# kerry-he/fsae-mpc

Hardware: AMD Instinct MI355X
Metric: QP solves/sec (batched LTV-MPC, N=40 nx=5 nu=2 fp64) (higher is better)
Workload: dtype f64

## Files before the change

### fsae-mpc_amd/csrc/qp_solve_kernel.h

```cpp
#pragma once
#include "qp_solver.h"
#include "qp_lane.h"

#ifndef QP_SOLVE_PAIR
#define QP_SOLVE_PAIR 0
#endif
#ifndef QP_DIAG_FLAT
#define QP_DIAG_FLAT 1
#endif
#ifndef QP_SYRK_INTERLEAVE
#define QP_SYRK_INTERLEAVE 0
#endif
#ifndef QP_STARTUP_ATW
#define QP_STARTUP_ATW 0
#endif

namespace {

template <int T> struct Tri {
  static constexpr int NT = T * (T + 1) / 2;
  __host__ __device__ static constexpr int idx(int I, int J) { return I * T - (I * (I - 1)) / 2 + (J - I); }
};

struct Ctx {
  int n, m, T, Kq, J, JB, JT, np, lane, c, q, nc, nb, ntr;
  const int* perm; const int* tcs; const int* aoff; const int* tend;
  const double* Aw; const double* Hw; const double* Ab; const double* Hb;
  double* rows;
  double* ring;
  double* cof;
  int rowlen;
  double* vec;
};
enum VecArr { V_X = 0, V_G, V_HX, V_R1, V_R2, V_P1, V_P2, V_P3, V_DX, V_E, V_NARR };

DEVINL double* rowp(const Ctx& k, int arr) { return k.rows + (size_t)arr * k.rowlen; }
DEVINL double* vecp(const Ctx& k, int arr) { return k.vec + arr * k.np; }

DEVINL bool row_valid(const Ctx& k, int js) {
  if (js < k.J) { const int s = 16 * js + k.c; return s < k.Kq && 4 * s + k.q < k.m; }
  return (js - k.J) * 64 + k.lane < k.n;
}

template <int T> DEVINL void hx_tiles(const Ctx& k, const double* X, double* HX) {
  double hx[T], hn[T][4], hc[T][4];
#pragma unroll
  for (int t = 0; t < T; ++t) hx[t] = 0.0;
#pragma unroll
  for (int Jt = 0; Jt < T; ++Jt)
#pragma unroll
    for (int p = 0; p < 4; ++p) hn[Jt][p] = k.Hw[((size_t)Jt * 4 + p) * 64 + k.lane];
#pragma unroll 1
  for (int I = 0; I < T; ++I) {
#pragma unroll
    for (int Jt = 0; Jt < T; ++Jt)
#pragma unroll
      for (int p = 0; p < 4; ++p) hc[Jt][p] = hn[Jt][p];
    if (I + 1 < T) {
#pragma unroll
      for (int Jt = 0; Jt < T; ++Jt)
#pragma unroll
        for (int p = 0; p < 4; ++p) hn[Jt][p] = k.Hw[((size_t)((I + 1) * T + Jt) * 4 + p) * 64 + k.lane];
    }
    double xk[4];
#pragma unroll
    for (int p = 0; p < 4; ++p) xk[p] = X[16 * I + k.q + 4 * p];
#pragma unroll
    for (int Jt = 0; Jt < T; ++Jt)
#pragma unroll
      for (int p = 0; p < 4; ++p) hx[Jt] = fma(hc[Jt][p], xk[p], hx[Jt]);
  }
#pragma unroll
  for (int t = 0; t < T; ++t) {
    double v = q_sum(hx[t]);
    if (k.q == 0) HX[16 * t + k.c] = v;
  }
}
template <int T> DEVINL void acc_init(const Ctx& k, v4d* acc) {
#pragma unroll
  for (int I = 0; I < T; ++I)
#pragma unroll
    for (int Jt = I; Jt < T; ++Jt) {
      const double* hp = k.Hw + ((size_t)(I * T + Jt) * 4) * 64 + k.lane;
      v4d h;
#pragma unroll
      for (int p = 0; p < 4; ++p) h[p] = hp[p * 64];
      acc[Tri<T>::idx(I, Jt)] = h;
    }
}

template <int T> DEVINL void hx_from_acc(const Ctx& k, const v4d* acc, const double* XV, double* HX) {
  double xr[T][4], xc[T], sc[T], sr[T][4];
#pragma unroll
  for (int I = 0; I < T; ++I) {
    xc[I] = XV[16 * I + k.c]; sc[I] = 0.0;
#pragma unroll
    for (int p = 0; p < 4; ++p) { xr[I][p] = XV[16 * I + k.q + 4 * p]; sr[I][p] = 0.0; }
  }
#pragma unroll
  for (int I = 0; I < T; ++I)
#pragma unroll
    for (int J = I; J < T; ++J) {
      const v4d& h = acc[Tri<T>::idx(I, J)];
#pragma unroll
      for (int p = 0; p < 4; ++p) {
        sc[J] = fma(h[p], xr[I][p], sc[J]);
        if (J > I) sr[I][p] = fma(h[p], xc[J], sr[I][p]);
      }
    }
  WAVE_SYNC();
#pragma unroll
  for (int J = 0; J < T; ++J) { const double v = q_sum(sc[J]); if (k.q == 0) HX[16 * J + k.c] = v; }
  WAVE_SYNC();
#pragma unroll
  for (int I = 0; I < T - 1; ++I) {
    grp16_sum(sr[I]);
#pragma unroll
    for (int p = 0; p < 4; ++p) if (k.c == 0) HX[16 * I + k.q + 4 * p] += sr[I][p];
  }
}

template <int C> struct IC { static constexpr int value = C; };

template <int T> struct StreamCfg {
  static constexpr int D = 2 * T;
  static constexpr int R = D + T;
};
template <int T> struct Stream {
  static constexpr int D = StreamCfg<T>::D, R = StreamCfg<T>::R;
  static_assert(R == QP_SOLVE_RING(T), "qp_solve_lds (qp_solver.h) sizes the ring");
  const char* gnext; int slot_i, slot_e;
  int tend[T + 1];
  DEVINL void issue(const Ctx& k) {
    __builtin_amdgcn_global_load_lds((const __attribute__((address_space(1))) void*)(gnext + k.lane * 16),
                                     (__attribute__((address_space(3))) void*)(k.ring + slot_i * 128), 16, 0, 0);
    gnext += 1024;
    slot_i = slot_i + 1 == R ? 0 : slot_i + 1;
  }
  DEVINL void open(const Ctx& k) {
    gnext = reinterpret_cast<const char*>(k.Aw); slot_i = 0; slot_e = 0;
#pragma unroll
    for (int C = 0; C <= T; ++C) tend[C] = uni(k.tend[C]);
  }
  DEVINL void start(const Ctx& k) {
    gnext = reinterpret_cast<const char*>(k.Aw); slot_i = 0; slot_e = 0;
    if (k.ntr > 0) {
#pragma unroll
      for (int j = 0; j < D; ++j) issue(k);
    }
#pragma unroll
    for (int C = 0; C <= T; ++C) tend[C] = uni(tend[C]);
  }
  template <int C> DEVINL void next_pair(const Ctx& k, v2d* b) {
#pragma unroll
    for (int t = 0; t < C; ++t) issue(k);
    asm volatile("s_waitcnt vmcnt(%0)" :: "n"(D) : "memory");
#pragma unroll
    for (int t = 0; t < C; ++t) {
      int sl = slot_e + t; if (sl >= R) sl -= R;
      b[t] = *reinterpret_cast<const v2d*>(k.ring + sl * 128 + k.lane * 2);
    }
    slot_e += C; if (slot_e >= R) slot_e -= R;
  }
  DEVINL void finish() { asm volatile("s_waitcnt vmcnt(0)" ::: "memory"); }
  DEVINL void close() { asm volatile("s_waitcnt vmcnt(0)" ::: "memory"); }
};

// ... 239 lines not shown
      double pv = q_sum(pc[t]);
      if (k.q == 0) Pcor[16 * t + k.c] = pv;
    }
#pragma unroll
    for (int f = 0; f < NB; ++f) { const double pv = q_sum(pcb[f]); if (k.lane == 0) Pcor[k.nc + f] = pv; }
  }
  if (FUSE >= 2) {
#pragma unroll
    for (int t = 0; t < T; ++t) {
      double pv = q_sum(pd[t]);
      if (k.q == 0) Pcor2[16 * t + k.c] = pv;
    }
#pragma unroll
    for (int f = 0; f < NB; ++f) { const double pv = q_sum(pdb[f]); if (k.lane == 0) Pcor2[k.nc + f] = pv; }
  }
}

template <int T, int NB> DEVINL void pass_Atw(const Ctx& k, const double* W, double* Pout) {
  constexpr int NBB = NB > 0 ? NB : 1;
  const int JS = k.J * 64;
  double p[T], pbv[NBB];
#pragma unroll
  for (int t = 0; t < T; ++t) p[t] = 0.0;
#pragma unroll
  for (int f = 0; f < NBB; ++f) pbv[f] = 0.0;
  for (int s = 0; s < 4 * k.ntr; ++s) {
    const int ri = (s >> 4) * 64 + k.q * 16 + (s & 15);
    const double w = W[ri];
    const int tr = s >> 2, tc = k.tcs[tr];
    const double* src = k.Aw + ((size_t)k.aoff[tr] + ((s >> 1) & 1) * tc) * 128 + k.lane * 2 + (s & 1);
#pragma unroll
    for (int t = 0; t < T; ++t)
      if (t < tc) p[t] = fma(w, src[t * 128], p[t]);
#pragma unroll
    for (int f = 0; f < NB; ++f) pbv[f] = fma(w, k.Ab[(size_t)f * JS + ri], pbv[f]);
  }
#pragma unroll
  for (int t = 0; t < T; ++t) {
    double v = q_sum(p[t]);
    if (k.q == 0) Pout[16 * t + k.c] = v;
  }
#pragma unroll
  for (int f = 0; f < NB; ++f) { const double pv = q_sum(pbv[f]); if (k.lane == 0) Pout[k.nc + f] = pv; }
}

template <int T> DEVINL void mfma4_sub(const v4d& X, const v4d& Y, v4d& Dst) {
#pragma unroll
  for (int p = 0; p < 4; ++p) Dst = __builtin_amdgcn_mfma_f64_16x16x4f64(-X[p], Y[p], Dst, 0, 0, 0);
}
DEVINL v4d mfma4_new(const v4d& X, const v4d& Y) {
  v4d Z = {0.0, 0.0, 0.0, 0.0};
#pragma unroll
  for (int p = 0; p < 4; ++p) Z = __builtin_amdgcn_mfma_f64_16x16x4f64(X[p], Y[p], Z, 0, 0, 0);
  return Z;
}

DEVINL void tile_store(const Ctx& k, double* slot, const v4d& Xt) {
#pragma unroll
  for (int p = 0; p < 4; ++p) slot[(k.q + 4 * p) * 17 + k.c] = Xt[p];
}
DEVINL v4d tile_load(const Ctx& k, const double* slot) {
  v4d Z;
#pragma unroll
  for (int p = 0; p < 4; ++p) Z[p] = slot[(k.q + 4 * p) * 17 + k.c];
  return Z;
}
DEVINL v4d tile_load_t(const Ctx& k, const double* slot) {
  v4d Z;
#pragma unroll
  for (int p = 0; p < 4; ++p) Z[p] = slot[k.c * 17 + k.q + 4 * p];
  return Z;
}

DEVINL double on_lanes(unsigned long long mask, double v, double otherwise) {
  return __builtin_amdgcn_inverse_ballot_w64(mask) ? v : otherwise;
}
template <int FORM> DEVINL int diag_factor(const Ctx& k, v4d& Ud, v4d& Yk, v4d& rk, double floor_abs) {
  constexpr bool FLAT = FORM >= 1;
  int bad = 0;
#pragma unroll
  for (int p = 0; p < 4; ++p) {
    const double d00 = rl(Ud[p], 4 * p + 0), d01 = rl(Ud[p], 4 * p + 1), d02 = rl(Ud[p], 4 * p + 2), d03 = rl(Ud[p], 4 * p + 3);
    const double d11 = rl(Ud[p], 16 + 4 * p + 1), d12 = rl(Ud[p], 16 + 4 * p + 2), d13 = rl(Ud[p], 16 + 4 * p + 3);
    const double d22 = rl(Ud[p], 32 + 4 * p + 2), d23 = rl(Ud[p], 32 + 4 * p + 3);
    const double d33 = rl(Ud[p], 48 + 4 * p + 3);
    auto piv = [&](double t) {
      if constexpr (FORM >= 2) {
        const bool low = !(t > floor_abs);
        bad |= (low & !(fabs(t) < INFINITY)) ? 1 : 0;
        t = low ? floor_abs : t;
      } else {
        if (!(t > floor_abs)) { if (!(fabs(t) < INFINITY)) bad = 1; t = floor_abs; }
      }
      return rsqrt(t);
    };
    const double i0 = piv(d00);
    const double r01 = d01 * i0, r02 = d02 * i0, r03 = d03 * i0;
    const double i1 = piv(fma(-r01, r01, d11));
    const double r12 = fma(-r01, r02, d12) * i1, r13 = fma(-r01, r03, d13) * i1;
    const double i2 = piv(fma(-r12, r12, fma(-r02, r02, d22)));
    const double r23 = fma(-r12, r13, fma(-r02, r03, d23)) * i2;
    const double i3 = piv(fma(-r23, r23, fma(-r13, r13, fma(-r03, r03, d33))));
    const double w10 = -r01 * i0 * i1;
    const double w20 = -fma(r12, w10, r02 * i0) * i2, w21 = -r12 * i1 * i2;
    const double w30 = -fma(r23, w20, fma(r13, w10, r03 * i0)) * i3, w31 = -fma(r23, w21, r13 * i1) * i3, w32 = -r23 * i2 * i3;
    const v4d z = {0.0, 0.0, 0.0, 0.0};
    if constexpr (FLAT) {
      const unsigned long long L0 = 1ull << (4 * p), L1 = 1ull << (16 + 4 * p), L2 = 1ull << (32 + 4 * p), L3 = 1ull << (48 + 4 * p);
      double wa = on_lanes(L0, i0, 0.0);
      wa = on_lanes(L0 << 1, w10, wa); wa = on_lanes(L0 << 2, w20, wa); wa = on_lanes(L0 << 3, w30, wa);
      wa = on_lanes(L1 << 1, i1, wa); wa = on_lanes(L1 << 2, w21, wa); wa = on_lanes(L1 << 3, w31, wa);
      wa = on_lanes(L2 << 2, i2, wa); wa = on_lanes(L2 << 3, w32, wa);
      wa = on_lanes(L3 << 3, i3, wa);
      const v4d nu = __builtin_amdgcn_mfma_f64_16x16x4f64(wa, Ud[p], z, 0, 0, 0);
      Ud[p] = nu[p];
      double a = 0.0;
      if (p < 3) {
        a = on_lanes(0x0001000100010001ull * (0xFFFFull & (0xFFFFull << (4 * p + 4))), -Ud[p], 0.0);
        Ud = __builtin_amdgcn_mfma_f64_16x16x4f64(a, Ud[p], Ud, 0, 0, 0);
      }
      const v4d ny = __builtin_amdgcn_mfma_f64_16x16x4f64(wa, Yk[p], z, 0, 0, 0);
      const v4d nr = __builtin_amdgcn_mfma_f64_16x16x4f64(wa, rk[p], z, 0, 0, 0);
      Yk[p] = ny[p]; rk[p] = nr[p];
      if (p < 3) {
        Yk = __builtin_amdgcn_mfma_f64_16x16x4f64(a, Yk[p], Yk, 0, 0, 0);
        rk = __builtin_amdgcn_mfma_f64_16x16x4f64(a, rk[p], rk, 0, 0, 0);
      }
      if constexpr (FORM >= 2) asm("" : "+v"(bad));
    } else {
      const int a_ = k.c - 4 * p;
      double wa = 0.0;
      if (k.q == 0) wa = a_ == 0 ? i0 : (a_ == 1 ? w10 : (a_ == 2 ? w20 : (a_ == 3 ? w30 : 0.0)));
      if (k.q == 1) wa = a_ == 1 ? i1 : (a_ == 2 ? w21 : (a_ == 3 ? w31 : 0.0));
      if (k.q == 2) wa = a_ == 2 ? i2 : (a_ == 3 ? w32 : 0.0);
      if (k.q == 3) wa = a_ == 3 ? i3 : 0.0;
      const v4d nu = __builtin_amdgcn_mfma_f64_16x16x4f64(wa, Ud[p], z, 0, 0, 0);
      const v4d ny = __builtin_amdgcn_mfma_f64_16x16x4f64(wa, Yk[p], z, 0, 0, 0);
      const v4d nr = __builtin_amdgcn_mfma_f64_16x16x4f64(wa, rk[p], z, 0, 0, 0);
      Ud[p] = nu[p]; Yk[p] = ny[p]; rk[p] = nr[p];
      if (p < 3) {
        const double a = (k.c > 4 * p + 3) ? -Ud[p] : 0.0;
        Yk = __builtin_amdgcn_mfma_f64_16x16x4f64(a, Yk[p], Yk, 0, 0, 0);
        rk = __builtin_amdgcn_mfma_f64_16x16x4f64(a, rk[p], rk, 0, 0, 0);
        Ud = __builtin_amdgcn_mfma_f64_16x16x4f64(a, Ud[p], Ud, 0, 0, 0);
      }
    }
  }
#pragma unroll
  for (int p = 0; p < 4; ++p) if (k.c < k.q + 4 * p) Ud[p] = 0.0;
  return bad;
}

template <int T, int NB> struct DiagForm { static constexpr int form = (T == 5 && NB > 0) ? QP_DIAG_FLAT : 0; };

template <int T, int NB, int K> struct FactorStep {
  static DEVINL int run(const Ctx& k, v4d* acc, double* YL, double floor_abs) {
    v4d Yk, none = {0.0, 0.0, 0.0, 0.0};
#pragma unroll
    for (int p = 0; p < 4; ++p) Yk[p] = (k.q + 4 * p == k.c) ? 1.0 : 0.0;
    int bad = diag_factor<DiagForm<T, NB>::form>(k, acc[Tri<T>::idx(K, K)], Yk, none, floor_abs);
    tile_store(k, YL + K * 272, Yk);
    WAVE_SYNC();
    const v4d Wk = tile_load_t(k, YL + K * 272);
    const v4d& UKK = acc[Tri<T>::idx(K, K)];
#pragma unroll
    for (int Jt = K + 1; Jt < T; ++Jt) {
      v4d Rr = acc[Tri<T>::idx(K, Jt)];
      v4d Ukj = mfma4_new(Wk, Rr);
      mfma4_sub<T>(UKK, Ukj, Rr);
#pragma unroll
      for (int p = 0; p < 4; ++p) Ukj = __builtin_amdgcn_mfma_f64_16x16x4f64(Wk[p], Rr[p], Ukj, 0, 0, 0);
      acc[Tri<T>::idx(K, Jt)] = Ukj;
    }
#pragma unroll
    for (int I = K + 1; I < T; ++I) {
      const v4d& UKI = acc[Tri<T>::idx(K, I)];
#pragma unroll
      for (int Jt = I; Jt < T; ++Jt) mfma4_sub<T>(UKI, acc[Tri<T>::idx(K, Jt)], acc[Tri<T>::idx(I, Jt)]);
    }
    return bad | FactorStep<T, NB, K + 1>::run(k, acc, YL, floor_abs);
  }
};
template <int T, int NB> struct FactorStep<T, NB, T> {
  static DEVINL int run(const Ctx&, v4d*, double*, double) { return 0; }
};
template <int T, int NB> DEVINL int reg_factor(const Ctx& k, v4d* acc, double* YL, double floor_abs) {
  return FactorStep<T, NB, 0>::run(k, acc, YL, floor_abs);
}

template <int T, bool REFINE, int NV> DEVINL void vec_forward(const Ctx& k, const v4d* acc, const double* YL, const double* const (&B)[NV], double (&y)[NV][T][4]) {
#pragma unroll
  for (int K = 0; K < T; ++K) {
    double s[NV], t[NV];
#pragma unroll
    for (int v = 0; v < NV; ++v) {
      s[v] = 0.0;
#pragma unroll
      for (int I = 0; I < K; ++I)
#pragma unroll
        for (int p = 0; p < 4; ++p) s[v] = fma(acc[Tri<T>::idx(I, K)][p], y[v][I][p], s[v]);
    }
    if (K > 0) q_sum(s);
#pragma unroll
    for (int v = 0; v < NV; ++v) t[v] = B[v][16 * K + k.c] - (K > 0 ? s[v] : 0.0);
    const v4d Yt = tile_load(k, YL + K * 272);
    double yk[NV * 4];
#pragma unroll
    for (int v = 0; v < NV; ++v)
#pragma unroll
      for (int p = 0; p < 4; ++p) yk[4 * v + p] = Yt[p] * t[v];
    grp16_sum(yk);
    if (REFINE) {
      const v4d& U = acc[Tri<T>::idx(K, K)];
      double r[NV], dy[NV * 4];
#pragma unroll
      for (int v = 0; v < NV; ++v) {
        r[v] = 0.0;
#pragma unroll
        for (int p = 0; p < 4; ++p) r[v] = fma(U[p], yk[4 * v + p], r[v]);
      }
      q_sum(r);
#pragma unroll
      for (int v = 0; v < NV; ++v) {
        r[v] = t[v] - r[v];
#pragma unroll
        for (int p = 0; p < 4; ++p) dy[4 * v + p] = Yt[p] * r[v];
      }
      grp16_sum(dy);
#pragma unroll
      for (int i = 0; i < NV * 4; ++i) yk[i] += dy[i];
    }
#pragma unroll
    for (int v = 0; v < NV; ++v)
#pragma unroll
      for (int p = 0; p < 4; ++p) y[v][K][p] = yk[4 * v + p];
  }
}
template <int T, bool REFINE> DEVINL void vec_forward(const Ctx& k, const v4d* acc, const double* YL, const double* B, double (&y)[T][4]) {
  const double* const b1[1] = {B};
  vec_forward<T, REFINE, 1>(k, acc, YL, b1, reinterpret_cast<double (&)[1][T][4]>(y));
}
template <int T, bool REFINE, int NV> DEVINL void vec_backward(const Ctx& k, const v4d* acc, const double* YL, const double (&y)[NV][T][4], double* const (&X)[NV]) {
  double x[NV][T];
#pragma unroll
  for (int K = T - 1; K >= 0; --K) {
    const v4d Yt = tile_load(k, YL + K * 272);
    double w[NV * 4], s[NV * 4], s2[NV];
#pragma unroll
    for (int v = 0; v < NV; ++v)
#pragma unroll
      for (int p = 0; p < 4; ++p) {
        s[4 * v + p] = 0.0;
#pragma unroll
        for (int J = K + 1; J < T; ++J) s[4 * v + p] = fma(acc[Tri<T>::idx(K, J)][p], x[v][J], s[4 * v + p]);
      }
    if (K < T - 1) grp16_sum(s);
#pragma unroll
    for (int v = 0; v < NV; ++v) {
      s2[v] = 0.0;
#pragma unroll
      for (int p = 0; p < 4; ++p) {
        w[4 * v + p] = y[v][K][p] - (K < T - 1 ? s[4 * v + p] : 0.0);
        s2[v] = fma(Yt[p], w[4 * v + p], s2[v]);
      }
    }
    q_sum(s2);
#pragma unroll
    for (int v = 0; v < NV; ++v) x[v][K] = s2[v];
    if (REFINE) {
      const v4d& U = acc[Tri<T>::idx(K, K)];
      double d[NV], ux[NV * 4];
#pragma unroll
      for (int v = 0; v < NV; ++v)
#pragma unroll
        for (int p = 0; p < 4; ++p) ux[4 * v + p] = U[p] * x[v][K];
      grp16_sum(ux);
#pragma unroll
      for (int v = 0; v < NV; ++v) {
        d[v] = 0.0;
#pragma unroll
        for (int p = 0; p < 4; ++p) d[v] = fma(Yt[p], w[4 * v + p] - ux[4 * v + p], d[v]);
      }
      q_sum(d);
#pragma unroll
      for (int v = 0; v < NV; ++v) x[v][K] += d[v];
    }
#pragma unroll
    for (int v = 0; v < NV; ++v) if (k.q == 0) X[v][16 * K + k.c] = x[v][K];
  }
}
template <int T, bool REFINE> DEVINL void vec_backward(const Ctx& k, const v4d* acc, const double* YL, const double (&y)[T][4], double* X) {
  double* const x1[1] = {X};
  vec_backward<T, REFINE, 1>(k, acc, YL, reinterpret_cast<const double (&)[1][T][4]>(y), x1);
}
template <int T> DEVINL void vec_rows_store(const Ctx& k, const double (&y)[T][4], double* V) {
  if (k.c == 0) {
#pragma unroll
    for (int K = 0; K < T; ++K)
#pragma unroll
      for (int p = 0; p < 4; ++p) V[16 * K + k.q + 4 * p] = y[K][p];
  }
}
template <int T> DEVINL void vec_rows_load(const Ctx& k, const double* V, double (&y)[T][4]) {
#pragma unroll
  for (int K = 0; K < T; ++K)
#pragma unroll
// ... 66 lines not shown
#define DX vecp(k, V_DX)
#define EV vecp(k, V_E)
#define aL rowp(k, R_L)
#define aU rowp(k, R_U)
#define aTL rowp(k, R_TL)
#define aTU rowp(k, R_TU)
#define aZL rowp(k, R_ZL)
#define aZU rowp(k, R_ZU)
#define aV rowp(k, R_V)
#define aD rowp(k, R_D)
#define aW1 rowp(k, R_W1)
#define aW2 rowp(k, R_W2)
#define aW3 rowp(k, R_W3)
#define aVA rowp(k, R_VA)
#define aVC rowp(k, R_VC)
#define aRPL rowp(k, R_RPL)
#define aRPU rowp(k, R_RPU)

  auto hx_border = [&](const double* XV) __attribute__((always_inline)) {
    if (NB > 0) {
      WAVE_SYNC();
      double xb[NBB], sb[NBB];
#pragma unroll
      for (int e = 0; e < NB; ++e) { xb[e] = XV[nc + e]; sb[e] = 0.0; }
      for (int h = 0; h < 2; ++h) {
        const int i = lane + 64 * h;
        if (i < n) {
          double add = 0.0;
#pragma unroll
          for (int e = 0; e < NB; ++e) { const double hbi = k.Hb[(size_t)e * k.np + i]; add = fma(hbi, xb[e], add); sb[e] = fma(hbi, XV[i], sb[e]); }
          if (i < nc) HX[i] += add;
        }
      }
      wave_sum(sb);
#pragma unroll
      for (int e = 0; e < NB; ++e) if (lane == 0) HX[nc + e] = sb[e];
    }
  };
  auto hx_full = [&](const double* XV) __attribute__((always_inline)) { hx_tiles<T>(k, XV, HX); hx_border(XV); };

  Stream<T> st;
  st.open(k);

  const double T0 = 10.0, Z0 = 100.0;
  for (int i = lane; i < k.np; i += 64) { G[i] = gw[i]; EV[i] = Es[i]; R1[i] = 0; R2[i] = 0; DX[i] = 0; }
  int cnt_local = 0, infeas = 0;
  for (int js = 0; js < JT; ++js) {
    const int ix = js * 64 + lane;
    const bool valid = row_valid(k, js);
    double l = aL[ix], u = aU[ix];
    if (valid) {
      if (l > -INFINITY && u < INFINITY) {
        if (l > u) infeas = 1;
        if (!(u > l)) {
          const double eps = 1e-9 * fmax(1.0, fabs(l));
          l -= eps; u += eps; aL[ix] = l; aU[ix] = u;
        }
      }
      cnt_local += (l > -INFINITY) + (u < INFINITY);
    }
    aW3[ix] = (valid && js < J) ? ((l > -INFINITY ? Z0 : 0.0) - (u < INFINITY ? Z0 : 0.0)) : 0.0;
    if (js >= J) {
      const int i = (js - J) * 64 + lane;
      if (i < k.np) {
        double xi = 0.0;
        if (P.x_init) { const int ui = i < k.n ? qp_user_index(d, i) : -1; if (ui >= 0) { const double xs = P.x_init[(size_t)b * d.nu + ui] / EV[i]; if (fabs(xs) < INFINITY) xi = xs; } }
        if (valid) { if (l > -INFINITY && xi < l) xi = l; if (u < INFINITY && xi > u) xi = u; }
        X[i] = xi;
      }
    }
  }
  const double cnt = fmax(1.0, wave_sum((double)cnt_local));
  infeas = wave_max((double)infeas) > 0;
  WAVE_SYNC();

  STAMP_DECL
  int flag = 1, it = 0, flag_polished = 0;
  double fval_s = 0.0, merit_s = INFINITY;
  if (infeas) { flag = -2; }
  if (ws[d.off_bad] != 0.0) flag = -1;

  {
    const double* vin[1] = {X}; double* rout[1] = {aV};
#if QP_STARTUP_ATW
    pass_Av<T, NB, 1, 0>(k, st, vin, rout, nullptr);
#else
    pass_Av<T, NB, 1, -1>(k, st, vin, rout, P3);
#endif
    for (int jb = 0; jb < k.JB; ++jb) { const int i = jb * 64 + lane; aV[(J + jb) * 64 + lane] = i < n ? X[i] : 0.0; }
  }
  STAMP_SETUP(2);
  for (int js = 0; js < JT; ++js) {
    const int ix = js * 64 + lane;
    const bool valid = row_valid(k, js);
    const double l = aL[ix], u = aU[ix], v = aV[ix];
    const bool hl = valid && l > -INFINITY, hu = valid && u < INFINITY;
    aTL[ix] = hl ? fmax(v - l, T0) : 1.0;
    aTU[ix] = hu ? fmax(u - v, T0) : 1.0;
    aZL[ix] = hl ? Z0 : 0.0;
    aZU[ix] = hu ? Z0 : 0.0;
  }
  WAVE_SYNC();
  STAMP_SETUP(3);
  {
    hx_full(X);
    STAMP_SETUP(4);
#if QP_STARTUP_ATW
    pass_Atw<T, NB>(k, aW3, P3);
#endif
    WAVE_SYNC();
    for (int jb = 0; jb < k.JB; ++jb) {
      const int i = jb * 64 + lane, ix = (J + jb) * 64 + lane;
      if (i < n) {
        const double r = HX[i] + G[i] - P3[i];
        if (aL[ix] > -INFINITY) aZL[ix] = fmax(r, 0.0) + Z0;
        if (aU[ix] < INFINITY) aZU[ix] = fmax(-r, 0.0) + Z0;
      }
    }
    WAVE_SYNC();
  }

  double saved_merit = INFINITY, best_res = INFINITY;
  int have_saved = 0, stall = 0;
  double* XS = ws + d.off_save;
  double* LAMS = ws + d.off_save + k.np;

  auto row1_body = [&](int ix, bool valid, double l, double u, double v, double tl, double tu, double zl, double zu,
                       double& s_gap, double& m_rp) {
    const bool hl = valid && l > -INFINITY, hu = valid && u < INFINITY;
    const double rpl = hl ? v - l - tl : 0.0, rpu = hu ? u - v - tu : 0.0;
    const double dl_ = hl ? zl / tl : 0.0, du_ = hu ? zu / tu : 0.0;
    aRPL[ix] = rpl; aRPU[ix] = rpu;
    rowp(k, R_CB1)[ix] = dl_; rowp(k, R_CC1)[ix] = hl ? dl_ / tl : 0.0;
    rowp(k, R_CB2)[ix] = du_; rowp(k, R_CC2)[ix] = hu ? du_ / tu : 0.0;
    aD[ix] = dl_ + du_;
    aW1[ix] = -dl_ * rpl + du_ * rpu;
    aW2[ix] = (hl ? 1.0 / tl : 0.0) - (hu ? 1.0 / tu : 0.0);
    aW3[ix] = (hl ? zl : 0.0) - (hu ? zu : 0.0);
    s_gap += (hl ? tl * zl : 0.0) + (hu ? tu * zu : 0.0);
    const double sc = fmax(1.0, fabs(v));
    if (hl) m_rp = fmax(m_rp, fabs(rpl) / fmax(sc, fabs(l)));
    if (hu) m_rp = fmax(m_rp, fabs(rpu) / fmax(sc, fabs(u)));
  };
  struct Slot { int ix; bool valid; double l, u, v, tl, tu, zl, zu, va, vc, w2, rpl, rpu; };
  auto load_slot = [&](int js) {
    Slot s_;
    const int jc = js < JT ? js : JT - 1;
    s_.ix = jc * 64 + lane; s_.valid = js < JT && row_valid(k, jc);
    const int ix = s_.ix;
    s_.l = aL[ix]; s_.u = aU[ix]; s_.v = aV[ix]; s_.tl = aTL[ix]; s_.tu = aTU[ix]; s_.zl = aZL[ix]; s_.zu = aZU[ix];
    s_.va = aVA[ix]; s_.vc = aVC[ix]; s_.w2 = aW2[ix]; s_.rpl = aRPL[ix]; s_.rpu = aRPU[ix];
    return s_;
  };
  double gap = 0.0, rp_rel = 0.0;

  v4d acc[NT];
  double Ubb[NBB][NBB];
  auto border_solve = [&](double* R) __attribute__((always_inline)) {
    if (NB > 0) {
      double yb[NBB], xb[NBB], dsum[NBB];
#pragma unroll
      for (int e = 0; e < NB; ++e) {
        dsum[e] = 0.0;
        for (int h = 0; h < 2; ++h) { const int i = lane + 64 * h; if (i < nc) dsum[e] = fma(MB[e * k.np + i], R[i], dsum[e]); }
      }
      wave_sum(dsum);
#pragma unroll
      for (int e = 0; e < NB; ++e) {
        double tt = R[nc + e] - dsum[e];
#pragma unroll
        for (int g2 = 0; g2 < e; ++g2) tt -= Ubb[g2][e] * yb[g2];
        yb[e] = tt / Ubb[e][e];
      }
#pragma unroll
      for (int e = NB - 1; e >= 0; --e) {
        double tt = yb[e];
#pragma unroll
        for (int f = e + 1; f < NB; ++f) tt -= Ubb[e][f] * xb[f];
        xb[e] = tt / Ubb[e][e];
      }
      WAVE_SYNC();
      for (int h = 0; h < 2; ++h) {
        const int i = lane + 64 * h;
        if (i < nc) {
          double r = R[i];
#pragma unroll
          for (int e = 0; e < NB; ++e) r = fma(-MB[e * k.np + i], xb[e], r);
          R[i] = r;
        }
      }
      if (lane == 0) {
#pragma unroll
        for (int e = 0; e < NB; ++e) R[nc + e] = xb[e];
      }
      WAVE_SYNC();
    }
  };
  auto factor_solve2 = [&](int it_now) __attribute__((always_inline)) -> int {
    double dmax_l = 0;
#pragma unroll
    for (int K = 0; K < T; ++K) {
      const int i = 16 * K + k.c;
      const int ix = (J + (i >> 6)) * 64 + (i & 63);
      const double dadd = i < n ? aD[ix] : 1.0;
      const bool mine = (k.q == (k.c & 3));
#pragma unroll
      for (int p = 0; p < 4; ++p)
        if (mine && p == (k.c >> 2)) { acc[Tri<T>::idx(K, K)][p] += dadd; dmax_l = fmax(dmax_l, acc[Tri<T>::idx(K, K)][p]); }
    }
    if (NB > 0) {
      for (int h = 0; h < 2; ++h) {
        const int i = lane + 64 * h;
        if (i < k.np) {
          const int ix = (J + (i >> 6)) * 64 + (i & 63);
#pragma unroll
          for (int e = 0; e < NB; ++e) {
            double v = i < n ? k.Hb[(size_t)e * k.np + i] + MB[e * k.np + i] : 0.0;
            if (i == nc + e) { v += e < nb ? aD[ix] : 1.0; dmax_l = fmax(dmax_l, v); }
            MB[e * k.np + i] = v;
          }
        }
      }
    }
    const double dmax = wave_max(dmax_l);
    WAVE_SYNC();
#ifdef QP_DEBUG_DUMP
    if (P.dump && b == 0 && P.dump_stage == 1 && it_now == P.dump_iter) {
#pragma unroll
      for (int I = 0; I < T; ++I)
#pragma unroll
        for (int Jt = I; Jt < T; ++Jt)
#pragma unroll
          for (int p = 0; p < 4; ++p) {
            const int r = 16 * I + k.q + 4 * p, cc = 16 * Jt + k.c;
            if (r < n && cc < n) { P.dump[r * n + cc] = acc[Tri<T>::idx(I, Jt)][p]; if (I != Jt || cc >= r) P.dump[cc * n + r] = acc[Tri<T>::idx(I, Jt)][p]; }
          }
      for (int e = 0; e < nb; ++e)
        for (int i = lane; i < n; i += 64) { P.dump[i * n + nc + e] = MB[e * k.np + i]; P.dump[(nc + e) * n + i] = MB[e * k.np + i]; }
      for (int i = lane; i < n; i += 64) { P.dump[n * n + i] = P1[i]; P.dump[n * n + n + i] = P2[i]; P.dump[n * n + 2 * n + i] = P3[i]; P.dump[n * n + 3 * n + i] = HX[i]; }
    }
#endif
    int fbad = reg_factor<T, NB>(k, acc, YL, 1e-30 * dmax);
    WAVE_SYNC();
    STAMP(5);
    if (NB > 0) {
#pragma unroll
      for (int e = 0; e < NB; ++e) {
        double ue[T][4];
        vec_forward<T, true>(k, acc, YL, MB + e * k.np, ue);
        WAVE_SYNC();
        vec_rows_store<T>(k, ue, MB + e * k.np);
      }
      WAVE_SYNC();
      double S[NBB][NBB], ss[NBB * (NBB + 1) / 2];
#pragma unroll
      for (int e = 0, j = 0; e < NB; ++e)
#pragma unroll
        for (int f = e; f < NB; ++f, ++j) {
          double dsum = 0.0;
          for (int h = 0; h < 2; ++h) { const int i = lane + 64 * h; if (i < nc) dsum = fma(MB[e * k.np + i], MB[f * k.np + i], dsum); }
          ss[j] = dsum;
        }
      wave_sum(ss);
#pragma unroll
      for (int e = 0, j = 0; e < NB; ++e)
#pragma unroll
        for (int f = e; f < NB; ++f, ++j) S[e][f] = MB[e * k.np + nc + f] - ss[j];
#pragma unroll
      for (int e = 0; e < NB; ++e) {
        double dd = S[e][e];
#pragma unroll
        for (int g2 = 0; g2 < e; ++g2) dd -= Ubb[g2][e] * Ubb[g2][e];
        if (!(dd > 1e-30 * dmax)) { if (!(fabs(dd) < INFINITY)) fbad = 1; dd = 1e-30 * dmax; }
        Ubb[e][e] = sqrt(dd);
#pragma unroll
        for (int f = e + 1; f < NB; ++f) {
          double tt = S[e][f];
#pragma unroll
          for (int g2 = 0; g2 < e; ++g2) tt -= Ubb[g2][e] * Ubb[g2][f];
          Ubb[e][f] = tt / Ubb[e][e];
        }
      }
    }
    if (fbad) return 1;
    {
      double y12[2][T][4];
      double (&y1)[T][4] = y12[0], (&y2)[T][4] = y12[1];
#if QP_SOLVE_PAIR
      { const double* const b12[2] = {R1, R2}; vec_forward<T, true, 2>(k, acc, YL, b12, y12); }
#else
      vec_forward<T, true>(k, acc, YL, R1, y1);
      vec_forward<T, true>(k, acc, YL, R2, y2);
#endif
      if (NB > 0) {
        WAVE_SYNC();
        vec_rows_store<T>(k, y1, R1); vec_rows_store<T>(k, y2, R2);
        WAVE_SYNC();
        border_solve(R1); border_solve(R2);
        vec_rows_load<T>(k, R1, y1); vec_rows_load<T>(k, R2, y2);
      }
      WAVE_SYNC();
#if QP_SOLVE_PAIR
      { double* const x12[2] = {R1, R2}; vec_backward<T, true, 2>(k, acc, YL, y12, x12); }
#else
      vec_backward<T, true>(k, acc, YL, y1, R1);
      vec_backward<T, true>(k, acc, YL, y2, R2);
#endif
    }
    WAVE_SYNC();
    return 0;
  };
  auto solve1 = [&](double* V) __attribute__((always_inline)) {
    double yv[T][4];
    vec_forward<T, false>(k, acc, YL, V, yv);
    if (NB > 0) {
      WAVE_SYNC();
      vec_rows_store<T>(k, yv, V);
      WAVE_SYNC();
      border_solve(V);
      vec_rows_load<T>(k, V, yv);
    }
    WAVE_SYNC();
    vec_backward<T, false>(k, acc, YL, yv, V);
  };

  STAMP(0);
  for (it = 0; flag == 1; ++it) {
    if (it == 0) {
      double s_gap = 0, m_rp = 0;
      for (int js = 0; js < JT; ++js) {
        const int ix = js * 64 + lane;
        row1_body(ix, row_valid(k, js), aL[ix], aU[ix], aV[ix], aTL[ix], aTU[ix], aZL[ix], aZU[ix], s_gap, m_rp);
      }
      gap = wave_sum(s_gap);
      rp_rel = wave_max(m_rp);
      WAVE_SYNC();
    }
    const double mu = gap / cnt;

    STAMP(1);
    acc_init<T>(k, acc);
    hx_from_acc<T>(k, acc, X, HX);
    hx_border(X);
    STAMP(2);
    pass_syrk<T, NB>(k, st, acc, P1, P2, P3, MB);
    WAVE_SYNC();
    STAMP(3);
    double fl = 0, m_rd = 0;
    for (int h = 0; h < 2; ++h) {
      const int i = lane + 64 * h;
      if (i < n) {
        const int ix = (J + (i >> 6)) * 64 + (i & 63);
        const double gz = P3[i] + aW3[ix];
        fl += 0.5 * X[i] * HX[i] + G[i] * X[i];
        const double sc = fmax(1.0, fmax(fabs(G[i]), fmax(fabs(HX[i]), fabs(gz))));
        m_rd = fmax(m_rd, fabs(HX[i] + G[i] - gz) / sc);
      }
    }
    const double fval = wave_sum(fl);
    const double rd_rel = wave_max(m_rd);
    const double gap_rel = gap / fmax(1.0, fabs(fval));
    const double merit = (fabs(fval) < INFINITY && fabs(gap_rel) < INFINITY) ? fmax(rd_rel, fmax(rp_rel, gap_rel)) : INFINITY;
    fval_s = fval; merit_s = merit;
    const bool res_ok = merit <= P.tol;
#ifdef QP_DEBUG_DUMP
    if (P.dump && P.dump_stage == 5 && b == P.dump_iter && lane == 0 && it < 120) {
      double* o_ = P.dump + 16 * it;
      o_[0] = merit; o_[1] = rd_rel; o_[2] = rp_rel; o_[3] = gap_rel; o_[4] = mu; o_[5] = fval; o_[6] = (double)have_saved; o_[7] = saved_merit;
    }
#endif
    if (!(merit < INFINITY)) { flag = have_saved ? 2 : -1; break; }
    if (merit <= P.tol_loose && merit < saved_merit) {
      for (int i = lane; i < k.np; i += 64) XS[i] = X[i];
      for (int js = 0; js < JT; ++js) LAMS[js * 64 + lane] = aW3[js * 64 + lane];
      have_saved = 1; saved_merit = merit;
    } else if (merit > P.tol_loose && rp_rel <= P.tol_loose && gap_rel <= P.tol_loose) {
      double dgap = 0, m_rd2 = 0, lamfix[2] = {0.0, 0.0};
      for (int h = 0; h < 2; ++h) {
        const int i = lane + 64 * h;
        if (i < n) {
          const int ix = (J + (i >> 6)) * 64 + (i & 63);
          const double lam = aW3[ix], gz = P3[i] + lam, r = HX[i] + G[i] - gz;
          const double lam2 = lam + r, l = aL[ix], u = aU[ix], v = aV[ix];
          const bool ok = lam2 >= 0 ? l > -INFINITY : u < INFINITY;
          if (ok) { lamfix[h] = lam2; dgap += fabs(r) * fmax(0.0, lam2 >= 0 ? v - l : u - v); }
          else {
            lamfix[h] = lam;
            const double sc = fmax(1.0, fmax(fabs(G[i]), fmax(fabs(HX[i]), fabs(gz))));
            m_rd2 = fmax(m_rd2, fabs(r) / sc);
          }
        }
      }
      const double merit2 = fmax(wave_max(m_rd2), fmax(rp_rel, (gap + wave_sum(dgap)) / fmax(1.0, fabs(fval))));
      if (merit2 <= P.tol_loose && merit2 < saved_merit) {
        for (int i = lane; i < k.np; i += 64) XS[i] = X[i];
        for (int js = 0; js < J; ++js) LAMS[js * 64 + lane] = aW3[js * 64 + lane];
        for (int h = 0; h < 2; ++h) { const int i = lane + 64 * h; if (i < k.np) LAMS[(J + (i >> 6)) * 64 + (i & 63)] = i < n ? lamfix[h] : 0.0; }
        have_saved = 1; saved_merit = merit2;
      }
      if (have_saved) { flag = 2; break; }
    } else if (have_saved && merit > P.tol_loose) { flag = 2; break; }
    if (merit < 0.9 * best_res) { best_res = merit; stall = 0; } else ++stall;

    for (int h = 0; h < 2; ++h) {
      const int i = lane + 64 * h;
      if (i < k.np) {
        const int ix = (J + (i >> 6)) * 64 + (i & 63);
        R1[i] = i < n ? -(HX[i] + G[i]) + P1[i] + aW1[ix] : 0.0;
        R2[i] = i < n ? P2[i] + aW2[ix] : 0.0;
      }
    }
    STAMP(4);
    if (factor_solve2(it)) {
      flag = (res_ok || have_saved) ? 2 : -1;
      if (flag == -1 && P.polish && rp_rel <= QP_BREAKDOWN_TRY_TOL && gap_rel <= QP_BREAKDOWN_TRY_TOL) flag = 4;
      break;
    }
    STAMP(6);
#ifdef QP_DEBUG_DUMP
    if (P.dump && b == 0 && P.dump_stage == 2 && it == P.dump_iter) {
      for (int i = lane; i < n; i += 64) { P.dump[i] = R1[i]; P.dump[n + i] = R2[i]; }
    }
#endif
    if (res_ok) {
      double dm = 0, xm = 1.0;
      for (int h = 0; h < 2; ++h) {
        const int i = lane + 64 * h;
        if (i < n) { dm = fmax(dm, fabs(R1[i] * EV[i])); xm = fmax(xm, fabs(X[i] * EV[i])); }
      }
      dm = wave_max(dm); xm = wave_max(xm);
      if (dm <= P.tol_x * xm) { flag = 0; break; }
    }
    if (it >= P.max_iter) { flag = have_saved ? 2 : 1; break; }

    {
      const double* vin[2] = {R1, R2}; double* rout[2] = {aVA, aVC};
      pass_Av<T, NB, 2, 1>(k, st, vin, rout, P1);
      for (int jb = 0; jb < k.JB; ++jb) {
        const int i = jb * 64 + lane;
        aVA[(J + jb) * 64 + lane] = i < n ? R1[i] : 0.0;
        aVC[(J + jb) * 64 + lane] = i < n ? R2[i] : 0.0;
      }
    }
    STAMP(7);
    double a_aff = 1.0, s1 = 0.0, s2 = 0.0;
    auto row2_body = [&](const Slot& r, int js) {
      const bool hl = r.valid && r.l > -INFINITY, hu = r.valid && r.u < INFINITY;
      double w = 0.0;
      if (hl) {
        const double dt = r.va + r.rpl, dz = -r.zl - (r.zl / r.tl) * dt;
        if (dt < 0) a_aff = fmin(a_aff, -r.tl / dt);
        if (dz < 0) a_aff = fmin(a_aff, -r.zl / dz);
        s1 += r.tl * dz + r.zl * dt; s2 += dt * dz;
        w -= dt * dz / r.tl;
      }
      if (hu) {
        const double dt = -r.va + r.rpu, dz = -r.zu - (r.zu / r.tu) * dt;
        if (dt < 0) a_aff = fmin(a_aff, -r.tu / dt);
        if (dz < 0) a_aff = fmin(a_aff, -r.zu / dz);
        s1 += r.tu * dz + r.zu * dt; s2 += dt * dz;
        w += dt * dz / r.tu;
      }
      if (js >= J && js < JT) aW1[r.ix] = w;
    };
    for (int js = 0; js < JT; js += 2) {
      const Slot r0 = load_slot(js), r1 = load_slot(js + 1);
      row2_body(r0, js); row2_body(r1, js + 1);
    }
    a_aff = wave_min(a_aff);
    s1 = wave_sum(s1); s2 = wave_sum(s2);
    const double mu_aff = fmax(0.0, gap + a_aff * (s1 + a_aff * s2)) / cnt;
    double sigma = mu > 0 ? (mu_aff / mu) * (mu_aff / mu) * (mu_aff / mu) : 0.0;
    if (sigma > 1.0) sigma = 1.0;
    {
      const double mu_floor = 1e-5 * P.tol * fmax(1.0, fabs(fval)) / cnt;
      if (mu > 0 && sigma < mu_floor / mu) sigma = fmin(1.0, mu_floor / mu);
    }
    const double smu = sigma * mu;
    const double cw = a_aff >= 0.05 ? 1.0 : 0.0;
    WAVE_SYNC();
    STAMP(8);
    if (cw != 0.0) {
    STAMP(9);
    for (int h = 0; h < 2; ++h) {
      const int i = lane + 64 * h;
      if (i < k.np) { const int ix = (J + (i >> 6)) * 64 + (i & 63); DX[i] = i < n ? P1[i] + aW1[ix] : 0.0; }
    }
    WAVE_SYNC();
    solve1(DX);
    WAVE_SYNC();
    STAMP(10);
    {
      const double* vin[1] = {DX}; double* rout[1] = {aW2};
      pass_Av<T, NB, 1, 0>(k, st, vin, rout, nullptr);
      for (int jb = 0; jb < k.JB; ++jb) { const int i = jb * 64 + lane; aW2[(J + jb) * 64 + lane] = i < n ? DX[i] : 0.0; }
    }
    STAMP(11);
    } else {
      for (int i = lane; i < k.np; i += 64) DX[i] = 0.0;
      for (int js = 0; js < JT; ++js) aW2[js * 64 + lane] = 0.0;
      WAVE_SYNC();
    }
    for (int h = 0; h < 2; ++h) {
      const int i = lane + 64 * h;
      if (i < n) DX[i] = R1[i] + smu * R2[i] + DX[i];
    }
    double amax = 1e300, bp = 0, bdp = 0, bd = 0, bdd = 0, q1 = 0.0, q2 = 0.0;
    auto row3a_body = [&](const Slot& r, int js) {
      const bool hl = r.valid && r.l > -INFINITY, hu = r.valid && r.u < INFINITY;
      const double dv = r.va + smu * r.vc + r.w2;
      if (js < JT) aVC[r.ix] = dv;
      if (hl) {
        const double dta = r.va + r.rpl, dza = -r.zl - (r.zl / r.tl) * dta;
        const double cl = smu - cw * dta * dza;
        const double dt = dv + r.rpl, dz = -r.zl + cl / r.tl - (r.zl / r.tl) * dt;
        if (dt < 0 && -r.tl / dt < amax) { amax = -r.tl / dt; bp = r.tl; bdp = dt; bd = r.zl; bdd = dz; }
        if (dz < 0 && -r.zl / dz < amax) { amax = -r.zl / dz; bp = r.zl; bdp = dz; bd = r.tl; bdd = dt; }
        q1 += r.tl * dz + r.zl * dt; q2 += dt * dz;
      }
      if (hu) {
        const double dta = -r.va + r.rpu, dza = -r.zu - (r.zu / r.tu) * dta;
        const double cu = smu - cw * dta * dza;
        const double dt = -dv + r.rpu, dz = -r.zu + cu / r.tu - (r.zu / r.tu) * dt;
        if (dt < 0 && -r.tu / dt < amax) { amax = -r.tu / dt; bp = r.tu; bdp = dt; bd = r.zu; bdd = dz; }
        if (dz < 0 && -r.zu / dz < amax) { amax = -r.zu / dz; bp = r.zu; bdp = dz; bd = r.tu; bdd = dt; }
        q1 += r.tu * dz + r.zu * dt; q2 += dt * dz;
      }
    };
    for (int js = 0; js < JT; js += 2) {
      const Slot r0 = load_slot(js), r1 = load_slot(js + 1);
      row3a_body(r0, js); row3a_body(r1, js + 1);
    }
    const double amax_w = wave_min(amax);
    double alpha = 1.0;
    if (amax_w < 1e299) {
      const unsigned long long msk = __ballot(amax == amax_w);
      const int src = __ffsll((long long)msk) - 1;
      bp = rl(bp, src); bdp = rl(bdp, src); bd = rl(bd, src); bdd = rl(bdd, src);
      q1 = wave_sum(q1); q2 = wave_sum(q2);
      const double gamma_f = 0.99, gamma_a = 1.0 / (1.0 - gamma_f);
      const double mufull = fmax(0.0, gap + amax_w * (q1 + amax_w * q2)) / cnt / gamma_a;
      const double a_h = (-bp + mufull / (bd + amax_w * bdd)) / bdp;
      alpha = fmin(1.0, fmin(0.99999999 * amax_w, fmax(a_h, gamma_f * amax_w)));
    }
#ifdef QP_DEBUG_DUMP
    if (P.dump && P.dump_stage == 5 && b == P.dump_iter && lane == 0 && it < 120) {
      double* o_ = P.dump + 16 * it;
      o_[8] = a_aff; o_[9] = sigma; o_[10] = alpha; o_[11] = cw; o_[12] = amax_w; o_[13] = (double)stall;
    }
    if (P.dump && b == 0 && P.dump_stage == 4 && it == P.dump_iter) {
      double c1 = 0, c2 = 0, c3 = 0, c4 = 0;
      for (int js = 0; js < JT; ++js) { const int ix = js * 64 + lane; c1 += aVA[ix]; c2 += aVC[ix]; c3 += aW2[ix]; c4 += aW1[ix]; }
      c1 = wave_sum(c1); c2 = wave_sum(c2); c3 = wave_sum(c3); c4 = wave_sum(c4);
      if (lane == 0) {
        double* o_ = P.dump;
        o_[0] = a_aff; o_[1] = mu_aff; o_[2] = sigma; o_[3] = smu; o_[4] = cw; o_[5] = amax_w; o_[6] = alpha; o_[7] = gap; o_[8] = mu;
        o_[9] = c1; o_[10] = c2; o_[11] = c3; o_[12] = c4; o_[13] = s1; o_[14] = s2; o_[15] = q1; o_[16] = q2;
      }
      for (int i = lane; i < n; i += 64) { P.dump[32 + i] = DX[i]; P.dump[32 + n + i] = R1[i]; P.dump[32 + 2 * n + i] = R2[i]; P.dump[32 + 3 * n + i] = P1[i]; }
    }
#endif
    double xn = 0, zn = 0, s_gap = 0, m_rp = 0;
    auto row3b_body = [&](const Slot& r, int js) {
      if (js >= JT) return;
      const bool hl = r.valid && r.l > -INFINITY, hu = r.valid && r.u < INFINITY;
      const double dv = r.vc;
      double tl = r.tl, zl = r.zl, tu = r.tu, zu = r.zu;
      if (hl) {
        const double dta = r.va + r.rpl, dza = -zl - (zl / tl) * dta;
        const double cl = smu - cw * dta * dza;
        const double dt = dv + r.rpl, dz = -zl + cl / tl - (zl / tl) * dt;
        tl += alpha * dt; zl += alpha * dz;
        aTL[r.ix] = tl; aZL[r.ix] = zl;
        zn = fmax(zn, zl);
      }
      if (hu) {
        const double dta = -r.va + r.rpu, dza = -zu - (zu / tu) * dta;
        const double cu = smu - cw * dta * dza;
        const double dt = -dv + r.rpu, dz = -zu + cu / tu - (zu / tu) * dt;
        tu += alpha * dt; zu += alpha * dz;
        aTU[r.ix] = tu; aZU[r.ix] = zu;
        zn = fmax(zn, zu);
      }
      const double v = r.v + alpha * dv;
      aV[r.ix] = v;
      row1_body(r.ix, r.valid, r.l, r.u, v, tl, tu, zl, zu, s_gap, m_rp);
    };
    for (int js = 0; js < JT; js += 2) {
      const Slot r0 = load_slot(js), r1 = load_slot(js + 1);
      row3b_body(r0, js); row3b_body(r1, js + 1);
    }
    for (int h = 0; h < 2; ++h) {
      const int i = lane + 64 * h;
      if (i < n) { X[i] += alpha * DX[i]; xn = fmax(xn, fabs(X[i])); }
    }
    const double rp_prev = rp_rel;
    gap = wave_sum(s_gap);
    rp_rel = wave_max(m_rp);
    xn = wave_max(xn); zn = wave_max(zn);
    WAVE_SYNC();
    STAMP(12);
    if (xn > 1e13) { flag = rp_prev > 1e-6 ? -2 : (fval < -1e13 ? -3 : -1); break; }
    if (zn > 1e15 && rp_prev > 1e-6) { flag = -2; break; }
    if (stall > (have_saved ? 5 : 25)) { flag = have_saved ? 2 : (rp_prev > 1e-6 ? -2 : (P.polish ? 5 : 1)); break; }
  }

  const bool v_current = flag == 0 || flag == 4;
  if (flag == 2) {
    for (int i = lane; i < k.np; i += 64) X[i] = XS[i];
    for (int js = 0; js < JT; ++js) aW3[js * 64 + lane] = LAMS[js * 64 + lane];
    flag = 0; merit_s = saved_merit;
    WAVE_SYNC();
  } else {
    for (int js = 0; js < JT; ++js) {
      const int ix = js * 64 + lane;
      const bool valid = row_valid(k, js);
      const bool hl = valid && aL[ix] > -INFINITY, hu = valid && aU[ix] < INFINITY;
      aW3[ix] = (hl ? aZL[ix] : 0.0) - (hu ? aZU[ix] : 0.0);
    }
    WAVE_SYNC();
  }
#ifdef QP_DEBUG_DUMP
  if (P.dump && P.dump_stage == 5 && b == P.dump_iter && lane == 0) { double* o_ = P.dump + 16 * 120; o_[4] = (double)flag; for (int i_ = 5; i_ < 48; ++i_) o_[i_] = 0.0; }
#endif
  if ((flag == 0 || flag == 4 || flag == 5) && P.polish) {
    const double rho = 1e6, pin = 1e16, rinv = 1.0 / rho;
    double* PA = rowp(k, R_CB1); double* PB = rowp(k, R_RPL); double* PY = rowp(k, R_CC1); double* PS = rowp(k, R_CB2);
    double* PC = rowp(k, R_RPU); double* PP = rowp(k, R_CC2); double* PZ0 = aW2;
    double* ATR = R1; double* ATP = P3;
    if (!v_current) {
      const double* vin[1] = {X}; double* rout[1] = {aV};
      pass_Av<T, NB, 1, 0>(k, st, vin, rout, nullptr);
      for (int jb = 0; jb < k.JB; ++jb) { const int i = jb * 64 + lane; aV[(J + jb) * 64 + lane] = i < n ? X[i] : 0.0; }
    }
    for (int js = 0; js < JT; ++js) {
      const int ix = js * 64 + lane;
      const bool valid = row_valid(k, js);
      const double l = aL[ix], u = aU[ix], v = aV[ix], lam = aW3[ix];
      const bool lo = valid && l > -INFINITY && lam > 0 && lam > fabs(v - l);
      const bool up = valid && u < INFINITY && lam < 0 && -lam > fabs(u - v);
      PS[ix] = lo ? 1.0 : (up ? -1.0 : 0.0); PY[ix] = ((lo || up) && js < J) ? lam : 0.0;
    }
    for (int i = lane; i < k.np; i += 64) XS[i] = X[i];
    WAVE_SYNC();
    for (int attempt = 0; attempt < QP_REFINE_ATTEMPTS && flag_polished <= 0; ++attempt) {
    for (int js = 0; js < JT; ++js) {
      const int ix = js * 64 + lane;
      const double sd = PS[ix];
      PA[ix] = sd != 0.0 ? rho : 0.0; PB[ix] = sd > 0 ? aL[ix] : (sd < 0 ? aU[ix] : 0.0);
      aD[ix] = js < J ? PA[ix] : (sd != 0.0 ? pin : 0.0); aW1[ix] = 0.0; aW2[ix] = 0.0; PC[ix] = 0.0; PP[ix] = 0.0;
    }
    WAVE_SYNC();
    acc_init<T>(k, acc);
    pass_syrk<T, NB>(k, st, acc, P1, P2, P3, MB);
    WAVE_SYNC();
    for (int i = lane; i < k.np; i += 64) { R1[i] = 0.0; R2[i] = 0.0; }
    WAVE_SYNC();
    bool pok = factor_solve2(-1) == 0, retry = false;
    if (!pok) { flag_polished = -5; break; }
    for (int h = 0; h < 2; ++h) {
      const int i = lane + 64 * h;
      if (i < k.np) { const int ix = (J + (i >> 6)) * 64 + (i & 63); R2[i] = (i < n && PS[ix] != 0.0) ? PB[ix] : XS[i]; }
    }
    WAVE_SYNC();
    const double* cf_eval[3] = {PA, PB, PY};
    const double* cf_cg[3] = {PA, PZ0, PZ0};
    auto eval_zy = [&]() __attribute__((always_inline)) {
      const double* vin[1] = {R2}; double* rout[2] = {aVA, aVC};
      pass_Av<T, NB, 1, 3>(k, st, vin, rout, P1, P2, cf_eval);
      hx_full(R2);
      WAVE_SYNC();
    };
    if (pok) {
      eval_zy();
      for (int h = 0; h < 2; ++h) {
        const int i = lane + 64 * h;
        if (i < k.np) { const int ix = (J + (i >> 6)) * 64 + (i & 63); DX[i] = (i < n && PS[ix] == 0.0) ? -(HX[i] + G[i] - P1[i]) : 0.0; }
      }
      WAVE_SYNC();
      solve1(DX);
      WAVE_SYNC();
      for (int h = 0; h < 2; ++h) {
        const int i = lane + 64 * h;
        if (i < n) { const int ix = (J + (i >> 6)) * 64 + (i & 63); if (PS[ix] == 0.0) R2[i] += DX[i]; }
      }
      WAVE_SYNC();
      eval_zy();
      double rs_l = 0.0;
      for (int js = 0; js < J; ++js) {
        const int ix = js * 64 + lane;
        const double cc_ = PA[ix] != 0.0 ? aVA[ix] - PB[ix] : 0.0;
        PC[ix] = cc_; PP[ix] = -cc_; rs_l = fma(cc_, cc_, rs_l);
      }
      double rs = wave_sum(rs_l);
      for (int h = 0; h < 2; ++h) { const int i = lane + 64 * h; if (i < k.np) { ATR[i] = -P2[i] * rinv; ATP[i] = ATR[i]; } }
      WAVE_SYNC();
      for (int cgit = 0; cgit < 12 && pok; ++cgit) {
        double m_eq = 0.0, m_cy = 0.0;
        for (int js = 0; js < J; ++js) {
          const int ix = js * 64 + lane;
          m_eq = fmax(m_eq, fabs(PC[ix]) / fmax(1.0, fabs(PB[ix])));
          m_cy = fmax(m_cy, fabs(PC[ix] * PY[ix]));
        }
        m_eq = wave_max(m_eq); m_cy = wave_max(m_cy);
        if (m_eq <= 1e-11 && m_cy <= 1e-11 * fmax(1.0, fabs(fval_s))) break;
        if (cgit == 11) { pok = false; flag_polished = -6; break; }
        for (int h = 0; h < 2; ++h) {
          const int i = lane + 64 * h;
          if (i < k.np) { const int ix = (J + (i >> 6)) * 64 + (i & 63); DX[i] = (i < n && PS[ix] == 0.0) ? ATP[i] : 0.0; }
        }
        WAVE_SYNC();
        solve1(DX);
        WAVE_SYNC();
        {
          const double* vin[1] = {DX}; double* rout[2] = {aVA, aVC};
          pass_Av<T, NB, 1, 3>(k, st, vin, rout, P1, P2, cf_cg);
        }
        WAVE_SYNC();
        double pq_l = 0.0;
        for (int js = 0; js < J; ++js) { const int ix = js * 64 + lane; if (PA[ix] != 0.0) pq_l = fma(PP[ix], aVA[ix], pq_l); }
        const double pq = wave_sum(pq_l);
        if (!(pq > 0.0) || !(rs > 0.0)) {
          pok = false; flag_polished = -7;
          if (attempt < QP_REFINE_ATTEMPTS - 1) {
            double my = 0.0; int myix = -1;
            for (int js = 0; js < J; ++js) { const int ix = js * 64 + lane; if (PA[ix] != 0.0 && fabs(PP[ix]) > my) { my = fabs(PP[ix]); myix = ix; } }
            const double mx = wave_max(my);
            if (mx > 0.0 && my == mx && myix >= 0) { PS[myix] = 0.0; PY[myix] = 0.0; }
            for (int i = lane; i < k.np; i += 64) XS[i] = R2[i];
            WAVE_SYNC();
            retry = true;
          }
          break;
        }
        const double alpha_ = rs / pq;
        double rsn_l = 0.0;
        for (int js = 0; js < J; ++js) {
          const int ix = js * 64 + lane;
          if (PA[ix] != 0.0) {
            PY[ix] = fma(alpha_, PP[ix], PY[ix]);
            const double cc_ = fma(alpha_, aVA[ix], PC[ix]);
            PC[ix] = cc_; rsn_l = fma(cc_, cc_, rsn_l);
          }
        }
// ... 195 lines not shown
```

Before: 433,700.

## Batch row sweeps and keep bound-row directions in registers

```diff
diff --git a/fsae-mpc_amd/csrc/qp_solve_kernel.h b/fsae-mpc_amd/csrc/qp_solve_kernel.h
--- a/fsae-mpc_amd/csrc/qp_solve_kernel.h
+++ b/fsae-mpc_amd/csrc/qp_solve_kernel.h
@@ -13,6 +13,9 @@
 #endif
 #ifndef QP_STARTUP_ATW
 #define QP_STARTUP_ATW 0
+#endif
+#ifndef QP_SWEEP_BATCH
+#define QP_SWEEP_BATCH 6
 #endif
 
 namespace {
@@ -558,6 +561,8 @@
 }
 
 template <int T, int NB> struct DiagForm { static constexpr int form = (T == 5 && NB > 0) ? QP_DIAG_FLAT : 0; };
+
+template <int T, int NB> struct SweepBatch { static constexpr int nsb = (T == 5 && NB > 0) ? QP_SWEEP_BATCH : 2; };
 
 template <int T, int NB, int K> struct FactorStep {
   static DEVINL int run(const Ctx& k, v4d* acc, double* YL, double floor_abs) {
@@ -930,6 +935,26 @@
     s_.va = aVA[ix]; s_.vc = aVC[ix]; s_.w2 = aW2[ix]; s_.rpl = aRPL[ix]; s_.rpu = aRPU[ix];
     return s_;
   };
+  struct BoundVals { double va[2], vc[2], w2[2]; };
+  auto bound_dirs = [&](BoundVals& bv) {
+    for (int h = 0; h < 2; ++h) { const int i = lane + 64 * h; bv.va[h] = i < n ? R1[i] : 0.0; bv.vc[h] = i < n ? R2[i] : 0.0; }
+  };
+  constexpr int NSB = SweepBatch<T, NB>::nsb;
+  auto sweep = [&](const BoundVals& bv, auto&& body) __attribute__((always_inline)) {
+    for (int js0 = 0; js0 < JT; js0 += NSB) {
+      Slot r[NSB];
+#pragma unroll
+      for (int e = 0; e < NSB; ++e) r[e] = load_slot(js0 + e);
+#pragma unroll
+      for (int e = 0; e < NSB; ++e) {
+        const int js = js0 + e;
+#pragma unroll
+        for (int h = 0; h < 2; ++h)
+          if (js == J + h) { r[e].va = bv.va[h]; r[e].vc = bv.vc[h]; r[e].w2 = bv.w2[h]; }
+        body(r[e], js);
+      }
+    }
+  };
   double gap = 0.0, rp_rel = 0.0;
 
   v4d acc[NT];
@@ -1124,12 +1149,15 @@
     pass_syrk<T, NB>(k, st, acc, P1, P2, P3, MB);
     WAVE_SYNC();
     STAMP(3);
-    double fl = 0, m_rd = 0;
+    double fl = 0, m_rd = 0, w1b[2] = {0.0, 0.0}, w2b[2] = {0.0, 0.0}, w3b[2] = {0.0, 0.0};
+    for (int h = 0; h < 2; ++h) {
+      const int i = lane + 64 * h;
+      if (i < n) { const int ix = (J + (i >> 6)) * 64 + (i & 63); w3b[h] = aW3[ix]; w1b[h] = aW1[ix]; w2b[h] = aW2[ix]; }
+    }
     for (int h = 0; h < 2; ++h) {
       const int i = lane + 64 * h;
       if (i < n) {
-        const int ix = (J + (i >> 6)) * 64 + (i & 63);
-        const double gz = P3[i] + aW3[ix];
+        const double gz = P3[i] + w3b[h];
         fl += 0.5 * X[i] * HX[i] + G[i] * X[i];
         const double sc = fmax(1.0, fmax(fabs(G[i]), fmax(fabs(HX[i]), fabs(gz))));
         m_rd = fmax(m_rd, fabs(HX[i] + G[i] - gz) / sc);
@@ -1183,9 +1211,8 @@
     for (int h = 0; h < 2; ++h) {
       const int i = lane + 64 * h;
       if (i < k.np) {
-        const int ix = (J + (i >> 6)) * 64 + (i & 63);
-        R1[i] = i < n ? -(HX[i] + G[i]) + P1[i] + aW1[ix] : 0.0;
-        R2[i] = i < n ? P2[i] + aW2[ix] : 0.0;
+        R1[i] = i < n ? -(HX[i] + G[i]) + P1[i] + w1b[h] : 0.0;
+        R2[i] = i < n ? P2[i] + w2b[h] : 0.0;
       }
     }
     STAMP(4);
@@ -1214,14 +1241,13 @@
     {
       const double* vin[2] = {R1, R2}; double* rout[2] = {aVA, aVC};
       pass_Av<T, NB, 2, 1>(k, st, vin, rout, P1);
-      for (int jb = 0; jb < k.JB; ++jb) {
-        const int i = jb * 64 + lane;
-        aVA[(J + jb) * 64 + lane] = i < n ? R1[i] : 0.0;
-        aVC[(J + jb) * 64 + lane] = i < n ? R2[i] : 0.0;
-      }
-    }
+    }
+    BoundVals bv;
+    bound_dirs(bv);
+    bv.w2[0] = bv.w2[1] = 0.0;
     STAMP(7);
     double a_aff = 1.0, s1 = 0.0, s2 = 0.0;
+    double wb[2] = {0.0, 0.0};
     auto row2_body = [&](const Slot& r, int js) {
       const bool hl = r.valid && r.l > -INFINITY, hu = r.valid && r.u < INFINITY;
       double w = 0.0;
@@ -1239,12 +1265,10 @@
         s1 += r.tu * dz + r.zu * dt; s2 += dt * dz;
         w += dt * dz / r.tu;
       }
-      if (js >= J && js < JT) aW1[r.ix] = w;
+      if (js == J) wb[0] = w;
+      if (js == J + 1) wb[1] = w;
     };
-    for (int js = 0; js < JT; js += 2) {
-      const Slot r0 = load_slot(js), r1 = load_slot(js + 1);
-      row2_body(r0, js); row2_body(r1, js + 1);
-    }
+    sweep(bv, row2_body);
     a_aff = wave_min(a_aff);
     s1 = wave_sum(s1); s2 = wave_sum(s2);
     const double mu_aff = fmax(0.0, gap + a_aff * (s1 + a_aff * s2)) / cnt;
@@ -1262,7 +1286,7 @@
     STAMP(9);
     for (int h = 0; h < 2; ++h) {
       const int i = lane + 64 * h;
-      if (i < k.np) { const int ix = (J + (i >> 6)) * 64 + (i & 63); DX[i] = i < n ? P1[i] + aW1[ix] : 0.0; }
+      if (i < k.np) DX[i] = i < n ? P1[i] + wb[h] : 0.0;
     }
     WAVE_SYNC();
     solve1(DX);
@@ -1271,23 +1295,27 @@
     {
       const double* vin[1] = {DX}; double* rout[1] = {aW2};
       pass_Av<T, NB, 1, 0>(k, st, vin, rout, nullptr);
-      for (int jb = 0; jb < k.JB; ++jb) { const int i = jb * 64 + lane; aW2[(J + jb) * 64 + lane] = i < n ? DX[i] : 0.0; }
     }
     STAMP(11);
     } else {
       for (int i = lane; i < k.np; i += 64) DX[i] = 0.0;
-      for (int js = 0; js < JT; ++js) aW2[js * 64 + lane] = 0.0;
+      for (int js = 0; js < J; ++js) aW2[js * 64 + lane] = 0.0;
       WAVE_SYNC();
     }
+    bound_dirs(bv);
+    for (int h = 0; h < 2; ++h) { const int i = lane + 64 * h; bv.w2[h] = i < n ? DX[i] : 0.0; }
     for (int h = 0; h < 2; ++h) {
       const int i = lane + 64 * h;
       if (i < n) DX[i] = R1[i] + smu * R2[i] + DX[i];
     }
     double amax = 1e300, bp = 0, bdp = 0, bd = 0, bdd = 0, q1 = 0.0, q2 = 0.0;
+    double dvb[2] = {0.0, 0.0};
     auto row3a_body = [&](const Slot& r, int js) {
       const bool hl = r.valid && r.l > -INFINITY, hu = r.valid && r.u < INFINITY;
       const double dv = r.va + smu * r.vc + r.w2;
-      if (js < JT) aVC[r.ix] = dv;
+      if (js < J) aVC[r.ix] = dv;
+      if (js == J) dvb[0] = dv;
+      if (js == J + 1) dvb[1] = dv;
       if (hl) {
         const double dta = r.va + r.rpl, dza = -r.zl - (r.zl / r.tl) * dta;
         const double cl = smu - cw * dta * dza;
@@ -1305,10 +1333,7 @@
         q1 += r.tu * dz + r.zu * dt; q2 += dt * dz;
       }
     };
-    for (int js = 0; js < JT; js += 2) {
-      const Slot r0 = load_slot(js), r1 = load_slot(js + 1);
-      row3a_body(r0, js); row3a_body(r1, js + 1);
-    }
+    sweep(bv, row3a_body);
     const double amax_w = wave_min(amax);
     double alpha = 1.0;
     if (amax_w < 1e299) {
@@ -1328,7 +1353,7 @@
     }
     if (P.dump && b == 0 && P.dump_stage == 4 && it == P.dump_iter) {
       double c1 = 0, c2 = 0, c3 = 0, c4 = 0;
-      for (int js = 0; js < JT; ++js) { const int ix = js * 64 + lane; c1 += aVA[ix]; c2 += aVC[ix]; c3 += aW2[ix]; c4 += aW1[ix]; }
+      for (int js = 0; js < J; ++js) { const int ix = js * 64 + lane; c1 += aVA[ix]; c2 += aVC[ix]; c3 += aW2[ix]; c4 += aW1[ix]; }
       c1 = wave_sum(c1); c2 = wave_sum(c2); c3 = wave_sum(c3); c4 = wave_sum(c4);
       if (lane == 0) {
         double* o_ = P.dump;
@@ -1364,10 +1389,8 @@
       aV[r.ix] = v;
       row1_body(r.ix, r.valid, r.l, r.u, v, tl, tu, zl, zu, s_gap, m_rp);
     };
-    for (int js = 0; js < JT; js += 2) {
-      const Slot r0 = load_slot(js), r1 = load_slot(js + 1);
-      row3b_body(r0, js); row3b_body(r1, js + 1);
-    }
+    bv.vc[0] = dvb[0]; bv.vc[1] = dvb[1];
+    sweep(bv, row3b_body);
     for (int h = 0; h < 2; ++h) {
       const int i = lane + 64 * h;
       if (i < n) { X[i] += alpha * DX[i]; xn = fmax(xn, fabs(X[i])); }
```

After: 440,000, median of 6. 1.4% higher.
